# ImIntheMiddle/VATL4Pose-WACV2024

Hardware: AMD Instinct MI355X
Metric: frames/sec pose-infer+uncertainty, 256x192 17-kp (higher is better)
Workload: dtype f32; 1 GPU; SimpleBaseline-R50 256x192 inference + decode + local-peak + THC-L1, 1024-frame synthetic video per GPU; frames_per_gpu=1024, batch=1024, tracks=4, parallelism=frame-sharded x1

## Files before the change

### vatl4pose-wacv2024_amd/csrc/winograd43.h

```cpp
#pragma once
#include "common.h"
#include "winograd_stage.h"

namespace vatl {

using W43Stage = WinoStage<3, 5>;
constexpr int W43_NLD = W43Stage::NLD;
constexpr int W43_LDS_BYTES = 2 * W43Stage::FLOATS * 4;
static_assert(W43Stage::NDMA % 4 == 0 && 16 * W_TB * 32 * 4 == W43_LDS_BYTES, "stage buffers = output-transform tiles");

__device__ __forceinline__ int w43_col_a(int nu) { return nu == 0 ? 0 : (nu == 2 ? 2 : 1); }
__device__ __forceinline__ int w43_col_b(int nu) { return nu == 0 ? 2 : (nu == 1 ? 2 : (nu == 2 ? 1 : 3)); }

template <int NP>
__device__ __forceinline__ void w43_make_v(f32x4 (&v)[5], const float* Rb, int ca, int cb, float sgn, int x8) {
    f32x4 tc[NP];
#pragma unroll
    for (int i = 0; i < NP; ++i) {
        const f32x4 da = *reinterpret_cast<const f32x4*>(Rb + i * W43Stage::ROWF + (ca ^ x8));
        const f32x4 db = *reinterpret_cast<const f32x4*>(Rb + i * W43Stage::ROWF + (cb ^ x8));
        tc[i] = da + sgn * db;
    }
    const f32x4 s = tc[3] - tc[1];
    v[0] = 2.f * (tc[0] - tc[2]) + s;
    v[1] = s - (tc[1] + tc[2]);
    v[2] = 2.f * tc[1] + (tc[3] - 3.f * tc[2]);
    v[3] = s;
    if constexpr (NP == 5) v[4] = (tc[4] - tc[2]) - 2.f * s;
}

template <int NP>
__device__ __forceinline__ void w43_mfma_group(f32x16 (&ac)[5], const f32x4 (&v)[5], const f32x4 (&uu)[5]) {
#pragma unroll
    for (int tt = 0; tt < 4; ++tt)
#pragma unroll
        for (int xi = 0; xi < NP; ++xi)
            ac[xi] = __builtin_amdgcn_mfma_f32_32x32x2f32(v[xi][tt], uu[xi][tt], ac[xi], 0, 0, 0);
}

typedef __int128 w43_count;
static inline bool w43_in_range(w43_count mt, w43_count xe, w43_count ye, w43_count ue, int Cin, int units) {
    return xe <= (w43_count)(WOOB_G / 4) && ye < ((w43_count)1 << 30) && ue < ((w43_count)1 << 28) && mt < ((w43_count)1 << 30) && Cin / W_CK < 1024 &&
           (mt + W_TB - 1) / W_TB * units < ((w43_count)1 << 31);
}

}
```

### vatl4pose-wacv2024_amd/csrc/winograd_deconv43.hip

```cpp
#include "common.h"
#include "buffer.h"
#include "tile_order.h"
#include "winograd43.h"

#include <algorithm>
#include <atomic>

namespace vatl {

struct Deconv43Params {
    const float* x;
    const float* u;
    const float* scale;
    const float* bias;
    float* y;
    int N, H, W, Cin, Cout;
    int TH, TW, tpi, Mtiles;
    int m_tiles, n_tiles;
    int relu;
    int stages;
    int rn;
    long long u_phase_floats;
    unsigned x_bytes, u_bytes, y_bytes;
    FastDivU d_TH, d_TW, d_tpi, d_grp, d_rn, d_rn_last, d_ntiles;
};

__device__ __forceinline__ void winograd_deconv43_body(const Deconv43Params& p, float* smem) {
    constexpr int NW = 4;
    float* Rs = smem;
    const int tid = threadIdx.x, lane = tid & 63, nu = __builtin_amdgcn_readfirstlane(tid >> 6);

    int m_tile, unit;
    grouped_tile(p, xcd_contiguous_index(blockIdx.x, gridDim.x), p.n_tiles * 4, m_tile, unit);
    const int phase = fdiv(unit, p.d_ntiles), n_tile = unit - phase * p.n_tiles;
    const int m0 = m_tile * W_TB, n0 = n_tile * 64;
    const int py = phase >> 1, px = phase & 1;
    const int pad_y = 1 - py, pad_x = 1 - px;

    const __amdgpu_buffer_rsrc_t xr = buf_rsrc(p.x, p.x_bytes);
    const __amdgpu_buffer_rsrc_t ur = buf_rsrc(p.u + (long long)phase * p.u_phase_floats, p.u_bytes);

    const int steps = p.stages * 2;
    const unsigned ubase = (unsigned)(((n_tile * steps) * 20 + nu) * 2 * 64 + lane) << 4;
    auto u_load = [&](f32x4 (&dst)[5], int step_, int half) {
        const int step = min(step_, steps - 1);
        const unsigned off = ubase + (unsigned)half * 1024u + (unsigned)step * 40960u;
#pragma unroll
        for (int xi = 0; xi < 5; ++xi) dst[xi] = buf_load4(ur, off + xi * 8192u);
    };
    f32x4 ua[5], ub[5];
    u_load(ua, 0, 0);

    unsigned goff[W43_NLD];
#pragma unroll
    for (int u = 0; u < W43_NLD; ++u)
        goff[u] = wino_piece_offset<W43Stage, 3, 4, false>(p, (nu + NW * u) * 64 + lane, m0, p.Mtiles, pad_y, pad_x, p.H, p.W);
    auto stage_dma = [&](int buf, int st) {
#pragma unroll
        for (int u = 0; u < W43_NLD; ++u)
            __builtin_amdgcn_raw_ptr_buffer_load_lds(xr, (lds_void*)(Rs + buf * W43Stage::FLOATS + (nu + NW * u) * 256), 16,
                                                     goff[u] + (unsigned)st * (W_CK * 4), 0, 0, 0);
    };
    stage_dma(0, 0);
    if (p.stages > 1) stage_dma(1, 1);

    const int h = lane >> 5;
    const float sgn = nu == 1 ? 1.f : -1.f;
    int ca, cb;
    {
        const int tl = lane & 31;
        const int m = min(m0 + tl, p.Mtiles - 1);
        const int gr = fdiv(m, p.d_TW), tx = m - gr * p.TW;
        ca = wino_frag_col<3>(w43_col_a(nu), tl, h, tx, pad_x, p.W);
        cb = wino_frag_col<3>(w43_col_b(nu), tl, h, tx, pad_x, p.W);
    }

    f32x16 accs[2][5];
#pragma unroll
    for (int hh = 0; hh < 2; ++hh)
#pragma unroll
        for (int xi = 0; xi < 5; ++xi)
#pragma unroll
            for (int e = 0; e < 16; ++e) accs[hh][xi][e] = 0.f;

    asm volatile("s_waitcnt vmcnt(0)" ::: "memory");
    __syncthreads();

    for (int st = 0; st < p.stages; ++st) {
        const int buf = st & 1;
        const float* Rb = Rs + buf * W43Stage::FLOATS;
        f32x4 v[5];
        u_load(ub, 2 * st, 1);
        __builtin_amdgcn_sched_barrier(0);
        w43_make_v<5>(v, Rb, ca, cb, sgn, 0);
        w43_mfma_group<5>(accs[0], v, ua);
        __builtin_amdgcn_sched_barrier(0);
        u_load(ua, 2 * st + 1, 0);
        __builtin_amdgcn_sched_barrier(0);
        w43_mfma_group<5>(accs[1], v, ub);
        __builtin_amdgcn_sched_barrier(0);
        u_load(ub, 2 * st + 1, 1);
        if (st + 1 < p.stages && st > 0) stage_dma(buf ^ 1, st + 1);
        __builtin_amdgcn_sched_barrier(0);
        w43_make_v<5>(v, Rb, ca, cb, sgn, 8);
        w43_mfma_group<5>(accs[0], v, ua);
        __builtin_amdgcn_sched_barrier(0);
        u_load(ua, 2 * st + 2, 0);
        __builtin_amdgcn_sched_barrier(0);
        w43_mfma_group<5>(accs[1], v, ub);
        __builtin_amdgcn_sched_barrier(0);
        asm volatile("s_waitcnt vmcnt(0)" ::: "memory");
        __syncthreads();
    }

    const __amdgpu_buffer_rsrc_t yr = buf_rsrc(p.y, p.y_bytes);
    const int c4 = tid & 7, tl = tid >> 3;
    const int OW = 2 * p.W;
    const unsigned cstep = (unsigned)(2 * p.Cout) << 2, rstep = (unsigned)(2 * OW * p.Cout) << 2;
    const bool valid = m0 + tl < p.Mtiles;
    unsigned obase;
    {
        const int m = min(m0 + tl, p.Mtiles - 1);
        const int b = fdiv(m, p.d_tpi), r = m - b * p.tpi;
        const int ty = fdiv(r, p.d_TW), tx = r - ty * p.TW;
        obase = (unsigned)(((b * 2 * p.H + 8 * ty + py) * OW + 6 * tx + px) * p.Cout + n0 + c4 * 4) << 2;
    }
    const float lo = p.relu ? 0.f : -INFINITY;
    float* Ps = smem;
#pragma unroll
    for (int hh = 0; hh < 2; ++hh) {
        const int n = n0 + 32 * hh + c4 * 4;
        f32x4 sc = {1.f, 1.f, 1.f, 1.f}, bi = {0.f, 0.f, 0.f, 0.f};
        if (p.scale) sc = *reinterpret_cast<const f32x4*>(p.scale + n);
        if (p.bias) bi = *reinterpret_cast<const f32x4*>(p.bias + n);
        {
            const int cl = lane & 31;
            f32x16 (&ac)[5] = accs[hh];
#pragma unroll
            for (int e = 0; e < 16; ++e) {
                const int row = (e & 3) + 8 * (e >> 2) + 4 * (lane >> 5);
                const float sum = ac[1][e] + ac[2][e], dif = ac[1][e] - ac[2][e], m3 = ac[3][e];
                Ps[((nu * 4 + 0) * W_TB + row) * 32 + cl] = ac[0][e] + sum + m3;
                Ps[((nu * 4 + 1) * W_TB + row) * 32 + cl] = dif + 2.f * m3;
                Ps[((nu * 4 + 2) * W_TB + row) * 32 + cl] = sum + 4.f * m3;
                Ps[((nu * 4 + 3) * W_TB + row) * 32 + cl] = dif + 8.f * m3 + ac[4][e];
            }
        }
        lds_barrier();
#pragma unroll
        for (int a = 0; a < 4; ++a) {
            f32x4 pq[4];
#pragma unroll
            for (int k = 0; k < 4; ++k) pq[k] = *reinterpret_cast<const f32x4*>(&Ps[((k * 4 + a) * W_TB + tl) * 32 + c4 * 4]);
            f32x4 yv[3];
            yv[0] = pq[0] + pq[1] + pq[2];
            yv[1] = pq[1] - pq[2];
            yv[2] = pq[1] + pq[2] + pq[3];
            if (valid) {
#pragma unroll
                for (int b = 0; b < 3; ++b) {
                    f32x4 o;
#pragma unroll
                    for (int c = 0; c < 4; ++c) o[c] = fmaxf(yv[b][c] * sc[c] + bi[c], lo);
                    buf_store4(yr, obase + (unsigned)hh * 128u + (unsigned)a * rstep + (unsigned)b * cstep, o);
                }
            }
        }
        if (hh == 0) lds_barrier();
    }
}

__global__ __launch_bounds__(256, 2) void winograd_deconv43_kernel(Deconv43Params p) {
    extern __shared__ __attribute__((aligned(16))) float smem[];
    winograd_deconv43_body(p, smem);
}

static std::atomic<unsigned> g_d43_lds_done;

}

using namespace vatl;

extern "C" int vatl_deconv4x4s2_winograd43_supported(int N, int H, int W, int Cin, int Cout) {
    if (N <= 0 || H <= 0 || W <= 0 || Cin <= 0 || Cout <= 0) return 0;
    if (H % 4 != 0 || W % 3 != 0 || Cin % 16 != 0 || Cout % 64 != 0) return 0;
    const w43_count n = N;
    return w43_in_range(n * (H / 4) * (W / 3), n * H * W * Cin, 4 * n * H * W * Cout, (w43_count)20 * Cout * Cin, Cin, Cout / 64 * 4) ? 1 : 0;
}

extern "C" int vatl_deconv4x4s2_winograd43_fwd(const float* x, const float* u, const float* scale, const float* bias, float* y, int N, int H, int W,
                                               int Cin, int Cout, int relu, void* stream) {
    if (!x || !u || !y) return fail(VATL_EINVAL, "deconv4x4s2_winograd43_fwd: null pointer");
    if (!vatl_deconv4x4s2_winograd43_supported(N, H, W, Cin, Cout))
        return fail(VATL_EINVAL, "deconv4x4s2_winograd43_fwd: %d x %dx%d x %d -> %d is outside H %% 4 == 0, W %% 3 == 0, Cin %% 16 == 0, Cout %% 64 == 0 and 32-bit offsets",
                    N, H, W, Cin, Cout);
    Deconv43Params p{};
    p.x = x; p.u = u; p.scale = scale; p.bias = bias; p.y = y;
    p.N = N; p.H = H; p.W = W; p.Cin = Cin; p.Cout = Cout; p.relu = relu;
    p.TH = H / 4; p.TW = W / 3; p.tpi = p.TH * p.TW;
    p.Mtiles = N * p.tpi;
    p.m_tiles = cdiv(p.Mtiles, W_TB);
    p.n_tiles = Cout / 64;
    p.stages = Cin / W_CK;
    p.u_phase_floats = 20LL * Cout * Cin;
    p.x_bytes = (unsigned)((long long)N * H * W * Cin * 4);
    p.y_bytes = (unsigned)(4LL * N * H * W * Cout * 4);
    p.u_bytes = (unsigned)(p.u_phase_floats * 4);
    const int units = p.n_tiles * 4;
    set_grouped_order(p, units, std::max(1, std::min(units, std::max(2, 2048 / (5 * Cin)))));
    p.d_TH = make_fastdiv(p.TH); p.d_TW = make_fastdiv(p.TW); p.d_tpi = make_fastdiv(p.tpi); p.d_ntiles = make_fastdiv(p.n_tiles);
    if (int rc = ensure_dynamic_lds((const void*)winograd_deconv43_kernel, W43_LDS_BYTES, g_d43_lds_done, "winograd_deconv43")) return rc;
    hipLaunchKernelGGL(winograd_deconv43_kernel, dim3((unsigned)(p.m_tiles * units)), dim3(256), W43_LDS_BYTES, (hipStream_t)stream, p);
    meter_add(1, 2.0 * ((double)p.m_tiles * W_TB) * 20.0 * (double)Cin * (double)Cout * 4.0);
    meter_route(kRouteWinoDeconv43);
    return check_launch("winograd_deconv43");
}
```

### vatl4pose-wacv2024_amd/csrc/winograd_s2_43.hip

```cpp
#include "common.h"
#include "buffer.h"
#include "tile_order.h"
#include "winograd43.h"

#include <algorithm>
#include <atomic>
#include <type_traits>

namespace vatl {

struct S2W43Params {
    const float* x;
    const float* u;
    const float* scale;
    const float* bias;
    float* y;
    int N, H, W, Cin, Cout;
    int OH, OW;
    int TH, TW, tpi, Mtiles;
    int m_tiles, n_tiles;
    int relu;
    int sp;
    int rn;
    unsigned x_bytes, u_bytes, y_bytes;
    FastDivU d_TH, d_TW, d_tpi, d_grp, d_rn, d_rn_last;
};

constexpr int S2W_ROW4_DMA = 4 * W43Stage::ROWE * 4 / 64;
static_assert(4 * W43Stage::ROWE * 4 % 64 == 0, "the fifth input row starts a DMA instruction");

__device__ __forceinline__ void winograd_s2_43_body(const S2W43Params& p, float* smem) {
    constexpr int NW = 4;
    float* Rs = smem;
    const int tid = threadIdx.x, lane = tid & 63, nu = __builtin_amdgcn_readfirstlane(tid >> 6);

    int m_tile, n_tile;
    grouped_tile(p, xcd_contiguous_index(blockIdx.x, gridDim.x), p.n_tiles, m_tile, n_tile);
    const int m0 = m_tile * W_TB, n0 = n_tile * 64;

    const __amdgpu_buffer_rsrc_t xr = buf_rsrc(p.x, p.x_bytes);
    const __amdgpu_buffer_rsrc_t ur = buf_rsrc(p.u, p.u_bytes);

    const int steps = p.sp * 2;
    const int gsteps = 4 * steps, gsteps5 = 2 * steps;
    const unsigned ubase = (unsigned)n_tile * (unsigned)steps * 147456u + ((unsigned)((nu * 2) * 64 + lane) << 4);
    auto u_load = [&](auto np, f32x4 (&dst)[5], int gstep_, int half) {
        constexpr int NP = decltype(np)::value;
        const int g = min(gstep_, gsteps - 1);
        const unsigned soff = g < gsteps5 ? (unsigned)g * 40960u : (unsigned)gsteps5 * 40960u + (unsigned)(g - gsteps5) * 32768u;
        const unsigned off = ubase + (unsigned)half * 1024u + soff;
#pragma unroll
        for (int xi = 0; xi < NP; ++xi) dst[xi] = buf_load4(ur, off + xi * 8192u);
    };
    f32x4 ua[5], ub[5];
    u_load(std::integral_constant<int, 5>{}, ua, 0, 0);

    unsigned goff[W43_NLD];
    auto set_goff = [&](int pad_y, int pad_x) {
        int m0 = m_tile * W_TB, ln = lane;
        asm volatile("" : "+s"(m0), "+v"(ln));
#pragma unroll
        for (int u = 0; u < W43_NLD; ++u) {
            __builtin_amdgcn_sched_barrier(0);
            goff[u] = wino_piece_offset<W43Stage, 3, 4, true>(p, (nu + NW * u) * 64 + ln, m0, p.Mtiles, pad_y, pad_x, p.OH, p.OW);
        }
    };
    auto stage_dma = [&](int buf, int st, bool rows5) {
        unsigned so = (unsigned)st * (W_CK * 4);
        asm volatile("" : "+s"(so));
#pragma unroll
        for (int u = 0; u < W43_NLD; ++u) {
            if (!rows5 && nu + NW * u >= S2W_ROW4_DMA) continue;
            __builtin_amdgcn_raw_ptr_buffer_load_lds(xr, (lds_void*)(Rs + buf * W43Stage::FLOATS + (nu + NW * u) * 256), 16,
                                                     goff[u] + so, 0, 0, 0);
        }
    };
    set_goff(1, 1);
    stage_dma(0, 0, true);

    const float sgn = nu == 1 ? 1.f : -1.f;
    int ca, cb;
    auto set_cols = [&](int pad_x) {
        int ln = lane;
        asm volatile("" : "+v"(ln));
        const int tl = ln & 31, h = ln >> 5;
        const int m = min(m0 + tl, p.Mtiles - 1);
        const int gr = fdiv(m, p.d_TW), tx = m - gr * p.TW;
        ca = wino_frag_col<3>(w43_col_a(nu), tl, h, tx, pad_x, p.OW);
        cb = wino_frag_col<3>(w43_col_b(nu), tl, h, tx, pad_x, p.OW);
    };

    f32x16 accs[2][5];
#pragma unroll
    for (int hh = 0; hh < 2; ++hh)
#pragma unroll
        for (int xi = 0; xi < 5; ++xi)
#pragma unroll
            for (int e = 0; e < 16; ++e) accs[hh][xi][e] = 0.f;

    asm volatile("s_waitcnt vmcnt(0)" ::: "memory");
    __syncthreads();

    auto run_phase = [&](auto np, int ph, int gs0) {
        constexpr int NP = decltype(np)::value;
        set_cols(1 - (ph & 1));
        for (int st = 0; st < p.sp; ++st) {
            const int gs = gs0 + st, buf = gs & 1;
            const float* Rb = Rs + buf * W43Stage::FLOATS;
            const bool wrap = st + 1 == p.sp;
            if (wrap && ph < 3) set_goff(1 - ((ph + 1) >> 1), 1 - ((ph + 1) & 1));
            f32x4 v[5];
            u_load(np, ub, 2 * gs, 1);
            __builtin_amdgcn_sched_barrier(0);
            w43_make_v<NP>(v, Rb, ca, cb, sgn, 0);
            w43_mfma_group<NP>(accs[0], v, ua);
            __builtin_amdgcn_sched_barrier(0);
            u_load(np, ua, 2 * gs + 1, 0);
            __builtin_amdgcn_sched_barrier(0);
            w43_mfma_group<NP>(accs[1], v, ub);
            __builtin_amdgcn_sched_barrier(0);
            u_load(np, ub, 2 * gs + 1, 1);
            if (!(wrap && ph == 3)) stage_dma(buf ^ 1, wrap ? 0 : st + 1, wrap ? ph + 1 < 2 : ph < 2);
            __builtin_amdgcn_sched_barrier(0);
            w43_make_v<NP>(v, Rb, ca, cb, sgn, 8);
            w43_mfma_group<NP>(accs[0], v, ua);
            __builtin_amdgcn_sched_barrier(0);
            u_load(np, ua, 2 * gs + 2, 0);
            __builtin_amdgcn_sched_barrier(0);
            w43_mfma_group<NP>(accs[1], v, ub);
            __builtin_amdgcn_sched_barrier(0);
            asm volatile("s_waitcnt vmcnt(0)" ::: "memory");
            __syncthreads();
        }
    };
    run_phase(std::integral_constant<int, 5>{}, 0, 0);
    run_phase(std::integral_constant<int, 5>{}, 1, p.sp);
    run_phase(std::integral_constant<int, 4>{}, 2, 2 * p.sp);
    run_phase(std::integral_constant<int, 4>{}, 3, 3 * p.sp);

    const __amdgpu_buffer_rsrc_t yr = buf_rsrc(p.y, p.y_bytes);
    const int c4 = tid & 7, tl = tid >> 3;
    const unsigned cstep = (unsigned)p.Cout << 2, rstep = (unsigned)(p.OW * p.Cout) << 2;
    const bool valid = m0 + tl < p.Mtiles;
    unsigned obase;
    {
        const int m = min(m0 + tl, p.Mtiles - 1);
        const int b = fdiv(m, p.d_tpi), r = m - b * p.tpi;
        const int ty = fdiv(r, p.d_TW), tx = r - ty * p.TW;
        obase = (unsigned)(((b * p.OH + 4 * ty) * p.OW + 3 * tx) * p.Cout + n0 + c4 * 4) << 2;
    }
    const float lo = p.relu ? 0.f : -INFINITY;
    float* Ps = smem;
#pragma unroll
    for (int hh = 0; hh < 2; ++hh) {
        const int n = n0 + 32 * hh + c4 * 4;
        f32x4 sc = {1.f, 1.f, 1.f, 1.f}, bi = {0.f, 0.f, 0.f, 0.f};
        if (p.scale) sc = *reinterpret_cast<const f32x4*>(p.scale + n);
        if (p.bias) bi = *reinterpret_cast<const f32x4*>(p.bias + n);
        {
            const int cl = lane & 31;
            f32x16 (&ac)[5] = accs[hh];
#pragma unroll
            for (int e = 0; e < 16; ++e) {
                const int row = (e & 3) + 8 * (e >> 2) + 4 * (lane >> 5);
                const float sum = ac[1][e] + ac[2][e], dif = ac[1][e] - ac[2][e], m3 = ac[3][e];
                Ps[((nu * 4 + 0) * W_TB + row) * 32 + cl] = ac[0][e] + sum + m3;
                Ps[((nu * 4 + 1) * W_TB + row) * 32 + cl] = dif + 2.f * m3;
                Ps[((nu * 4 + 2) * W_TB + row) * 32 + cl] = sum + 4.f * m3;
                Ps[((nu * 4 + 3) * W_TB + row) * 32 + cl] = dif + 8.f * m3 + ac[4][e];
            }
        }
        lds_barrier();
#pragma unroll
        for (int a = 0; a < 4; ++a) {
            f32x4 pq[4];
#pragma unroll
            for (int k = 0; k < 4; ++k) pq[k] = *reinterpret_cast<const f32x4*>(&Ps[((k * 4 + a) * W_TB + tl) * 32 + c4 * 4]);
            f32x4 yv[3];
            yv[0] = pq[0] + pq[1] + pq[2];
            yv[1] = pq[1] - pq[2];
            yv[2] = pq[1] + pq[2] + pq[3];
            if (valid) {
#pragma unroll
                for (int b = 0; b < 3; ++b) {
                    f32x4 o;
#pragma unroll
                    for (int c = 0; c < 4; ++c) o[c] = fmaxf(yv[b][c] * sc[c] + bi[c], lo);
                    buf_store4(yr, obase + (unsigned)hh * 128u + (unsigned)a * rstep + (unsigned)b * cstep, o);
                }
            }
        }
        if (hh == 0) lds_barrier();
    }
}

__global__ __launch_bounds__(256, 2) void winograd_s2_43_kernel(S2W43Params p) {
    extern __shared__ __attribute__((aligned(16))) float smem[];
    winograd_s2_43_body(p, smem);
}

static std::atomic<unsigned> g_s2w43_lds_done;

}

using namespace vatl;

extern "C" int vatl_conv3x3s2_winograd43_supported(int N, int H, int W, int Cin, int Cout) {
    if (N <= 0 || H <= 0 || W <= 0 || Cin <= 0 || Cout <= 0) return 0;
    if (H % 8 != 0 || W % 6 != 0 || Cin % 16 != 0 || Cout % 64 != 0) return 0;
    const w43_count n = N;
    return w43_in_range(n * (H / 8) * (W / 6), n * H * W * Cin, n * (H / 2) * (W / 2) * Cout, (w43_count)72 * Cout * Cin, Cin, Cout / 64) ? 1 : 0;
}

extern "C" int vatl_conv3x3s2_winograd43_fwd(const float* x, const float* u, const float* scale, const float* bias, float* y, int N, int H, int W,
                                             int Cin, int Cout, int relu, void* stream) {
    if (!x || !u || !y) return fail(VATL_EINVAL, "conv3x3s2_winograd43_fwd: null pointer");
    if (!vatl_conv3x3s2_winograd43_supported(N, H, W, Cin, Cout))
        return fail(VATL_EINVAL, "conv3x3s2_winograd43_fwd: %d x %dx%d x %d -> %d is outside H %% 8 == 0, W %% 6 == 0, Cin %% 16 == 0, Cout %% 64 == 0 and 32-bit offsets",
                    N, H, W, Cin, Cout);
    S2W43Params p{};
    p.x = x; p.u = u; p.scale = scale; p.bias = bias; p.y = y;
    p.N = N; p.H = H; p.W = W; p.Cin = Cin; p.Cout = Cout; p.relu = relu;
    p.OH = H / 2; p.OW = W / 2;
    p.TH = p.OH / 4; p.TW = p.OW / 3; p.tpi = p.TH * p.TW;
    p.Mtiles = N * p.tpi;
    p.m_tiles = cdiv(p.Mtiles, W_TB);
    p.n_tiles = Cout / 64;
    p.sp = Cin / W_CK;
    p.x_bytes = (unsigned)((long long)N * H * W * Cin * 4);
    p.y_bytes = (unsigned)((long long)N * p.OH * p.OW * Cout * 4);
    p.u_bytes = (unsigned)(72LL * Cout * Cin * 4);
    set_grouped_order(p, p.n_tiles, std::max(1, std::min(p.n_tiles, std::max(2, 2048 / (18 * Cin)))));
    p.d_TH = make_fastdiv(p.TH); p.d_TW = make_fastdiv(p.TW); p.d_tpi = make_fastdiv(p.tpi);
    if (int rc = ensure_dynamic_lds((const void*)winograd_s2_43_kernel, W43_LDS_BYTES, g_s2w43_lds_done, "winograd_s2_43")) return rc;
    hipLaunchKernelGGL(winograd_s2_43_kernel, dim3((unsigned)(p.m_tiles * p.n_tiles)), dim3(256), W43_LDS_BYTES, (hipStream_t)stream, p);
    meter_add(0, 2.0 * ((double)p.m_tiles * W_TB) * 72.0 * (double)Cin * (double)Cout);
    meter_route(kRouteWinoS2_43);
    return check_launch("winograd_s2_43");
}
```

Measured before the change: 17730 frames/s.

## Use counted vmcnt waits to keep U-operand loads in flight across stages

Replaces compiler-managed buffer loads of the Winograd U operand with inline-asm requests and explicit partial s_waitcnt vmcnt(N) waits, so each MFMA group waits only for its own operand rather than draining all outstanding memory ops at stage end. The per-stage loop body is factored into a shared w43_stage helper. The LDS DMA is now issued unconditionally every stage, with a zero-size buffer descriptor or out-of-bounds offset standing in for the skipped loads, which keeps vmcnt counts uniform. The final stage barrier waits only for the prefetched next-stage operands. This relies on exact in-order vmcnt accounting; any miscount would read stale registers or LDS.

```diff
diff --git a/vatl4pose-wacv2024_amd/csrc/winograd43.h b/vatl4pose-wacv2024_amd/csrc/winograd43.h
--- a/vatl4pose-wacv2024_amd/csrc/winograd43.h
+++ b/vatl4pose-wacv2024_amd/csrc/winograd43.h
@@ -38,6 +38,51 @@
             ac[xi] = __builtin_amdgcn_mfma_f32_32x32x2f32(v[xi][tt], uu[xi][tt], ac[xi], 0, 0, 0);
 }
 
+
+template <int NP>
+__device__ __forceinline__ void w43_request(f32x4 (&dst)[5], __amdgpu_buffer_rsrc_t r, unsigned voff, unsigned soff) {
+#pragma unroll
+    for (int xi = 0; xi < NP; ++xi)
+        asm volatile("buffer_load_dwordx4 %0, %1, %2, %3 offen" : "=&v"(dst[xi]) : "v"(voff), "s"(r), "s"(soff + xi * 8192u));
+}
+
+template <int N>
+__device__ __forceinline__ void w43_wait(f32x4 (&u)[5]) {
+    asm volatile("s_waitcnt vmcnt(%5)" : "+v"(u[0]), "+v"(u[1]), "+v"(u[2]), "+v"(u[3]), "+v"(u[4]) : "n"(N) : "memory");
+}
+
+template <int NP, class ULoad, class StageDma>
+__device__ __forceinline__ void w43_stage(f32x16 (&accs)[2][5], f32x4 (&ua)[5], f32x4 (&ub)[5], const float* Rb, int ca, int cb, float sgn, int s0,
+                                          ULoad&& u_load, StageDma&& stage_dma) {
+    constexpr int F = NP, FD = NP + W43_NLD;
+    f32x4 v[5];
+    u_load(ub, s0, 1);
+    __builtin_amdgcn_sched_barrier(0);
+    w43_make_v<NP>(v, Rb, ca, cb, sgn, 0);
+    w43_wait<F>(ua);
+    w43_mfma_group<NP>(accs[0], v, ua);
+    __builtin_amdgcn_sched_barrier(0);
+    u_load(ua, s0 + 1, 0);
+    __builtin_amdgcn_sched_barrier(0);
+    w43_wait<F>(ub);
+    w43_mfma_group<NP>(accs[1], v, ub);
+    __builtin_amdgcn_sched_barrier(0);
+    u_load(ub, s0 + 1, 1);
+    stage_dma();
+    __builtin_amdgcn_sched_barrier(0);
+    w43_make_v<NP>(v, Rb, ca, cb, sgn, 8);
+    w43_wait<FD>(ua);
+    w43_mfma_group<NP>(accs[0], v, ua);
+    __builtin_amdgcn_sched_barrier(0);
+    u_load(ua, s0 + 2, 0);
+    __builtin_amdgcn_sched_barrier(0);
+    w43_wait<FD>(ub);
+    w43_mfma_group<NP>(accs[1], v, ub);
+    __builtin_amdgcn_sched_barrier(0);
+    w43_wait<F>(ua);
+    lds_barrier();
+}
+
 typedef __int128 w43_count;
 static inline bool w43_in_range(w43_count mt, w43_count xe, w43_count ye, w43_count ue, int Cin, int units) {
     return xe <= (w43_count)(WOOB_G / 4) && ye < ((w43_count)1 << 30) && ue < ((w43_count)1 << 28) && mt < ((w43_count)1 << 30) && Cin / W_CK < 1024 &&
diff --git a/vatl4pose-wacv2024_amd/csrc/winograd_deconv43.hip b/vatl4pose-wacv2024_amd/csrc/winograd_deconv43.hip
--- a/vatl4pose-wacv2024_amd/csrc/winograd_deconv43.hip
+++ b/vatl4pose-wacv2024_amd/csrc/winograd_deconv43.hip
@@ -44,9 +44,7 @@
     const unsigned ubase = (unsigned)(((n_tile * steps) * 20 + nu) * 2 * 64 + lane) << 4;
     auto u_load = [&](f32x4 (&dst)[5], int step_, int half) {
         const int step = min(step_, steps - 1);
-        const unsigned off = ubase + (unsigned)half * 1024u + (unsigned)step * 40960u;
-#pragma unroll
-        for (int xi = 0; xi < 5; ++xi) dst[xi] = buf_load4(ur, off + xi * 8192u);
+        w43_request<5>(dst, ur, ubase, (unsigned)half * 1024u + (unsigned)step * 40960u);
     };
     f32x4 ua[5], ub[5];
     u_load(ua, 0, 0);
@@ -55,14 +53,13 @@
 #pragma unroll
     for (int u = 0; u < W43_NLD; ++u)
         goff[u] = wino_piece_offset<W43Stage, 3, 4, false>(p, (nu + NW * u) * 64 + lane, m0, p.Mtiles, pad_y, pad_x, p.H, p.W);
-    auto stage_dma = [&](int buf, int st) {
+    auto stage_dma = [&](__amdgpu_buffer_rsrc_t r, int buf, int st) {
 #pragma unroll
         for (int u = 0; u < W43_NLD; ++u)
-            __builtin_amdgcn_raw_ptr_buffer_load_lds(xr, (lds_void*)(Rs + buf * W43Stage::FLOATS + (nu + NW * u) * 256), 16,
+            __builtin_amdgcn_raw_ptr_buffer_load_lds(r, (lds_void*)(Rs + buf * W43Stage::FLOATS + (nu + NW * u) * 256), 16,
                                                      goff[u] + (unsigned)st * (W_CK * 4), 0, 0, 0);
     };
-    stage_dma(0, 0);
-    if (p.stages > 1) stage_dma(1, 1);
+    stage_dma(xr, 0, 0);
 
     const int h = lane >> 5;
     const float sgn = nu == 1 ? 1.f : -1.f;
@@ -83,35 +80,16 @@
 #pragma unroll
             for (int e = 0; e < 16; ++e) accs[hh][xi][e] = 0.f;
 
-    asm volatile("s_waitcnt vmcnt(0)" ::: "memory");
+    w43_wait<0>(ua);
     __syncthreads();
 
     for (int st = 0; st < p.stages; ++st) {
         const int buf = st & 1;
-        const float* Rb = Rs + buf * W43Stage::FLOATS;
-        f32x4 v[5];
-        u_load(ub, 2 * st, 1);
-        __builtin_amdgcn_sched_barrier(0);
-        w43_make_v<5>(v, Rb, ca, cb, sgn, 0);
-        w43_mfma_group<5>(accs[0], v, ua);
-        __builtin_amdgcn_sched_barrier(0);
-        u_load(ua, 2 * st + 1, 0);
-        __builtin_amdgcn_sched_barrier(0);
-        w43_mfma_group<5>(accs[1], v, ub);
-        __builtin_amdgcn_sched_barrier(0);
-        u_load(ub, 2 * st + 1, 1);
-        if (st + 1 < p.stages && st > 0) stage_dma(buf ^ 1, st + 1);
-        __builtin_amdgcn_sched_barrier(0);
-        w43_make_v<5>(v, Rb, ca, cb, sgn, 8);
-        w43_mfma_group<5>(accs[0], v, ua);
-        __builtin_amdgcn_sched_barrier(0);
-        u_load(ua, 2 * st + 2, 0);
-        __builtin_amdgcn_sched_barrier(0);
-        w43_mfma_group<5>(accs[1], v, ub);
-        __builtin_amdgcn_sched_barrier(0);
-        asm volatile("s_waitcnt vmcnt(0)" ::: "memory");
-        __syncthreads();
+        const bool more = st + 1 < p.stages;
+        w43_stage<5>(accs, ua, ub, Rs + buf * W43Stage::FLOATS, ca, cb, sgn, 2 * st, u_load,
+                     [&] { stage_dma(more ? xr : buf_rsrc(p.x, 0), buf ^ 1, st + 1); });
     }
+    w43_wait<0>(ua);
 
     const __amdgpu_buffer_rsrc_t yr = buf_rsrc(p.y, p.y_bytes);
     const int c4 = tid & 7, tl = tid >> 3;
diff --git a/vatl4pose-wacv2024_amd/csrc/winograd_s2_43.hip b/vatl4pose-wacv2024_amd/csrc/winograd_s2_43.hip
--- a/vatl4pose-wacv2024_amd/csrc/winograd_s2_43.hip
+++ b/vatl4pose-wacv2024_amd/csrc/winograd_s2_43.hip
@@ -48,9 +48,7 @@
         constexpr int NP = decltype(np)::value;
         const int g = min(gstep_, gsteps - 1);
         const unsigned soff = g < gsteps5 ? (unsigned)g * 40960u : (unsigned)gsteps5 * 40960u + (unsigned)(g - gsteps5) * 32768u;
-        const unsigned off = ubase + (unsigned)half * 1024u + soff;
-#pragma unroll
-        for (int xi = 0; xi < NP; ++xi) dst[xi] = buf_load4(ur, off + xi * 8192u);
+        w43_request<NP>(dst, ur, ubase, (unsigned)half * 1024u + soff);
     };
     f32x4 ua[5], ub[5];
     u_load(std::integral_constant<int, 5>{}, ua, 0, 0);
@@ -62,18 +60,17 @@
 #pragma unroll
         for (int u = 0; u < W43_NLD; ++u) {
             __builtin_amdgcn_sched_barrier(0);
-            goff[u] = wino_piece_offset<W43Stage, 3, 4, true>(p, (nu + NW * u) * 64 + ln, m0, p.Mtiles, pad_y, pad_x, p.OH, p.OW);
-        }
-    };
-    auto stage_dma = [&](int buf, int st, bool rows5) {
+            if (pad_y == 0 && nu + NW * u >= S2W_ROW4_DMA) goff[u] = WOOB_G;
+            else goff[u] = wino_piece_offset<W43Stage, 3, 4, true>(p, (nu + NW * u) * 64 + ln, m0, p.Mtiles, pad_y, pad_x, p.OH, p.OW);
+        }
+    };
+    auto stage_dma = [&](int buf, int st, bool fetch) {
         unsigned so = (unsigned)st * (W_CK * 4);
         asm volatile("" : "+s"(so));
-#pragma unroll
-        for (int u = 0; u < W43_NLD; ++u) {
-            if (!rows5 && nu + NW * u >= S2W_ROW4_DMA) continue;
-            __builtin_amdgcn_raw_ptr_buffer_load_lds(xr, (lds_void*)(Rs + buf * W43Stage::FLOATS + (nu + NW * u) * 256), 16,
-                                                     goff[u] + so, 0, 0, 0);
-        }
+        const __amdgpu_buffer_rsrc_t r = buf_rsrc(p.x, fetch ? p.x_bytes : 0u);
+#pragma unroll
+        for (int u = 0; u < W43_NLD; ++u)
+            __builtin_amdgcn_raw_ptr_buffer_load_lds(r, (lds_void*)(Rs + buf * W43Stage::FLOATS + (nu + NW * u) * 256), 16, goff[u] + so, 0, 0, 0);
     };
     set_goff(1, 1);
     stage_dma(0, 0, true);
@@ -98,7 +95,7 @@
 #pragma unroll
             for (int e = 0; e < 16; ++e) accs[hh][xi][e] = 0.f;
 
-    asm volatile("s_waitcnt vmcnt(0)" ::: "memory");
+    w43_wait<0>(ua);
     __syncthreads();
 
     auto run_phase = [&](auto np, int ph, int gs0) {
@@ -106,37 +103,17 @@
         set_cols(1 - (ph & 1));
         for (int st = 0; st < p.sp; ++st) {
             const int gs = gs0 + st, buf = gs & 1;
-            const float* Rb = Rs + buf * W43Stage::FLOATS;
             const bool wrap = st + 1 == p.sp;
             if (wrap && ph < 3) set_goff(1 - ((ph + 1) >> 1), 1 - ((ph + 1) & 1));
-            f32x4 v[5];
-            u_load(np, ub, 2 * gs, 1);
-            __builtin_amdgcn_sched_barrier(0);
-            w43_make_v<NP>(v, Rb, ca, cb, sgn, 0);
-            w43_mfma_group<NP>(accs[0], v, ua);
-            __builtin_amdgcn_sched_barrier(0);
-            u_load(np, ua, 2 * gs + 1, 0);
-            __builtin_amdgcn_sched_barrier(0);
-            w43_mfma_group<NP>(accs[1], v, ub);
-            __builtin_amdgcn_sched_barrier(0);
-            u_load(np, ub, 2 * gs + 1, 1);
-            if (!(wrap && ph == 3)) stage_dma(buf ^ 1, wrap ? 0 : st + 1, wrap ? ph + 1 < 2 : ph < 2);
-            __builtin_amdgcn_sched_barrier(0);
-            w43_make_v<NP>(v, Rb, ca, cb, sgn, 8);
-            w43_mfma_group<NP>(accs[0], v, ua);
-            __builtin_amdgcn_sched_barrier(0);
-            u_load(np, ua, 2 * gs + 2, 0);
-            __builtin_amdgcn_sched_barrier(0);
-            w43_mfma_group<NP>(accs[1], v, ub);
-            __builtin_amdgcn_sched_barrier(0);
-            asm volatile("s_waitcnt vmcnt(0)" ::: "memory");
-            __syncthreads();
+            w43_stage<NP>(accs, ua, ub, Rs + buf * W43Stage::FLOATS, ca, cb, sgn, 2 * gs, [&](f32x4 (&dst)[5], int g, int half) { u_load(np, dst, g, half); },
+                          [&] { stage_dma(buf ^ 1, wrap ? 0 : st + 1, !(wrap && ph == 3)); });
         }
     };
     run_phase(std::integral_constant<int, 5>{}, 0, 0);
     run_phase(std::integral_constant<int, 5>{}, 1, p.sp);
     run_phase(std::integral_constant<int, 4>{}, 2, 2 * p.sp);
     run_phase(std::integral_constant<int, 4>{}, 3, 3 * p.sp);
+    w43_wait<0>(ua);
 
     const __amdgpu_buffer_rsrc_t yr = buf_rsrc(p.y, p.y_bytes);
     const int c4 = tid & 7, tl = tid >> 3;
```

Result: no change. 17800 frames/s, median of 6 (+0.4%).
